# edantec/MPC_benchmark

Hardware: AMD Instinct MI355X
Metric: mpc_solves_per_sec (higher is better)
Workload: dtype f64

## Files before the change

### mpc_benchmark_amd/csrc/layout.h

```cpp
#pragma once
#include <stdint.h>

struct Layout {
  int N, B, space, nx, n, m, c, nz;
  int nj;
  int model_mask_off;
  int oH, oG, oAB, oF, oE6, oT6k, oD12, oCV, oCD, oLO, oHI, oDT, oACT, oCT, oMISC, oXD, oWR, oXN, knot_stride;
  int oP, op, oK, ok, oKnu, oknu, oMx, omx, oT6, oPhi, ophi, gain_stride;
  int oMu, oZnu, oGam, oKu, oKnup, oLm, mpad;
  int lSg, lsg, lZx, lzc, lcP, lcp, lth, ldP, leg_stride;
  int tP, tLm, tSg, tZx, tZt, tF, tE, tp, tsg, tzc, tu, txin, ttho, tree_stride;
  int wPh, wPt, wLp, wG, wHh, wgh, wCt, wW, wY, wSc, wV, wAcl, wvec, work_stride;
  int max_stage_ints, max_stage_doubles;
  int n_alpha;
  int sc_cap;
};

enum { MISC_COST = 0, MISC_PEN = 1, MISC_PRIM = 2, MISC_NC = 3, MISC_M = 4, MISC_DUAL = 5, MISC_CRIT = 6, MISC_DMERIT = 7, MISC_COUNT = 8 };

struct InstState {
  double mu, inner_tol, prim_tol;
  double phi0, dphi0, alpha, cost, prim, dual, crit;
  int32_t num_iters, al_iters, converged, done, skip_step, ls_step, ls_more, stalled;
  int32_t corrector, pad_;
// ... 6 lines not shown
static inline void make_layout(Layout& L) {
  const int n = L.n, m = L.m, c = L.c, nz = L.nz = n + m;
  int o = 0;
  auto take = [&](int cnt) { int r = o; o += align2(cnt); return r; };
  L.oH = take(nz * nz); L.oG = take(nz); L.oAB = take(n * nz); L.oF = take(n); L.oE6 = take(36); L.oT6k = take(36);
  L.oD12 = take(74);
  L.oCV = take(c); L.oCD = take(c * nz); L.oLO = take(c); L.oHI = take(c); L.oDT = take(c); L.oACT = take(c); L.oCT = take(c);
  L.oMISC = take(MISC_COUNT); L.oXD = take(n); L.oWR = take(12); L.oXN = take(L.nx);
  L.knot_stride = o;
  o = 0;
  L.oP = take(n * n); L.op = take(n); L.oK = take(m * n); L.ok = take(m); L.oKnu = take(c * n); L.oknu = take(c);
  L.oMx = take(n * n); L.omx = take(n); L.oT6 = take(36);
  L.oPhi = take(n * n); L.ophi = take(n);
  L.mpad = (m + 15) & ~15;
  L.oMu = take(L.mpad * L.mpad); L.oZnu = take(c * L.mpad); L.oGam = take(n * n); L.oKu = take(m * n); L.oKnup = take(c * n); L.oLm = take(n * n);
  L.gain_stride = o;
  o = 0;
  L.lSg = take(n * n); L.lsg = take(n); L.lZx = take(n * n); L.lzc = take(n); L.lcP = take(n * n); L.lcp = take(n); L.lth = take(n); L.ldP = take(n * n);
  L.leg_stride = o;
  o = 0;
  L.tP = take(n * n); L.tLm = take(n * n); L.tSg = take(n * n); L.tZx = take(n * n); L.tZt = take(n * n); L.tF = take(n * n); L.tE = take(n * n);
  L.tp = take(n); L.tsg = take(n); L.tzc = take(n); L.tu = take(n); L.txin = take(n); L.ttho = take(n);
  L.tree_stride = o;
  o = 0;
  const int nr = n + 1;
  L.wPh = take(n * n); L.wPt = take(n * n); L.wLp = take(n * n); L.wG = take(n * nz); L.wHh = take(nz * nz); L.wgh = take(nz);
  L.wCt = take(c * nz); L.wW = take(m * nr); L.wY = take(m * c); L.wSc = take(c * c); L.wV = take(c * nr); L.wAcl = take(n * nr);
  L.wvec = take(8 * (nz + c));
  L.work_stride = o;
  L.sc_cap = c < 48 ? c : 48;
// ... 2 lines not shown
```

### mpc_benchmark_amd/csrc/legs.h

```cpp
#pragma once
#include "mfma_blocks.h"
#include "solver_kernels.h"

#define LEG_BARRIER() asm volatile("s_waitcnt lgkmcnt(0)\n\ts_barrier" ::: "memory")

#define LEG_LAUNDER() do { asm volatile("" : "+v"(tid), "+v"(lane)); wv = __builtin_amdgcn_readfirstlane(tid >> 6); } while (0)

#define LK_THREADS 512
#define LK_U 20
#define LK_PT 13
#define LK_TILES 5

struct LkLds {
  int np, mp, nzp, lda, ldp, ldm, nb, nbm;
  int AB, PR, TM, ZN, vec, total_bytes;
  unsigned mg_nzp, mg_np, mg_mp;
};
static inline constexpr LkLds make_lk_lds(int n, int m) {
  LkLds s{};
  s.np = (n + 15) & ~15; s.mp = (m + 15) & ~15; s.nzp = s.np + s.mp; s.lda = s.nzp + 1; s.ldp = s.np + 1; s.ldm = s.mp + 1;
  s.nb = s.np / 16; s.nbm = s.mp / 16;
  s.mg_nzp = magic_div(s.nzp); s.mg_np = magic_div(s.np); s.mg_mp = magic_div(s.mp);
  int o = 0;
  auto take = [&](int cnt) { int r = o; o += (cnt + 1) & ~1; return r; };
  const int pr = s.np * s.ldp > s.mp * s.np + s.mp * s.ldm ? s.np * s.ldp : s.mp * s.np + s.mp * s.ldm;
  s.AB = take(s.np * s.lda); s.PR = take(pr); s.TM = take(6 * s.nzp + 6 * s.np + 40); s.ZN = take(16 * s.ldm); s.vec = take(s.mp + 3 * s.np + 80 + 8);
  s.total_bytes = o * 8;
  return s;
}

template <int MP, int FN = 0, int FM = 0>
DEV void leg_knot_body(const SolverArgs& a, const LkLds& Srt, const int b, const int kbeg, const int kend, const int prof_b, const int prof_k) {
  constexpr bool FX = FN > 0;
  constexpr LkLds SC_ = FX ? make_lk_lds(FN, FM) : LkLds{};
  LkLds S_ = Srt;
  if constexpr (FX) S_ = SC_;
  const LkLds& S = S_;
  constexpr int NAB = (80 * (80 + MP) + LK_THREADS - 1) / LK_THREADS, NK = (MP * 80 + LK_THREADS - 1) / LK_THREADS;
  constexpr int NMU = (MP * MP + LK_THREADS - 1) / LK_THREADS, NZN = (16 * MP + LK_THREADS - 1) / LK_THREADS;
  const Layout& L = a.L;
  int tid = threadIdx.x, lane = tid & 63;
  constexpr int nthr = LK_THREADS, nw = LK_THREADS / 64;
  int wv = __builtin_amdgcn_readfirstlane(tid >> 6);
  const InstState& st = a.inst[b];
  if (st.done || st.skip_step) return;
  const int n = FX ? FN : L.n, nz = FX ? FN + FM : L.nz, np = S.np, mp = S.mp, nzp = S.nzp, lda = S.lda, ldp = S.ldp, ldm = S.ldm, nb = S.nb, nbm = S.nbm;
  const double mud = st.mu * a.opt.dyn_al_scale;
  extern __shared__ __attribute__((aligned(16))) double sm[];
  double *AB = sm + S.AB, *PR = sm + S.PR, *ZN = sm + S.ZN, *vec = sm + S.vec;
  double *KM = PR, *PT = PR, *U1 = PR, *MU = PR + mp * np;
  double *TMP = sm + S.TM, *PT6 = TMP + 6 * nzp, *c6 = PT6 + 6 * np;
  double *kf = vec, *y0 = vec + mp, *z0 = y0 + np, *t6 = z0 + np, *g6 = t6 + 36, *mxs = g6 + 36;
  int* cnt = (int*)(mxs + np);
  long long tk0_ = clock64();
#define LK_PROF(slot) do { if (a.prof && k == prof_k && b == prof_b && tid == 0) { const long long t1_ = clock64(); a.prof[prof_b * 64 + 32 + (slot)] += (double)(t1_ - tk0_); tk0_ = t1_; } } while (0)

  double pab[NAB], pkm[NK], ptv[LK_PT], pmu[NMU], pzn[NZN], psm = 0.0, pact = 0.0;
  auto request_ab = [&](int k) {
    const double* kn = knot_ptr(a, b, k);
    const double* g = gain_ptr(a, b, k);
    const int m = (int)kn[L.oMISC + MISC_M], c = (int)kn[L.oMISC + MISC_NC];
#pragma unroll
    for (int u = 0; u < NAB; ++u) {
      const int idx = tid + u * nthr, i = qdiv(idx, S.mg_nzp), zp = (idx - qdiv(idx, S.mg_nzp) * nzp);
      const int z = (zp < n) ? zp : ((zp >= np && zp - np < m) ? n + zp - np : -1);
      pab[u] = (idx < np * nzp && i < n && z >= 0) ? kn[L.oAB + (size_t)i * nz + z] : 0.0;
    }
#pragma unroll
    for (int u = 0; u < NK; ++u) {
      const int idx = tid + u * nthr, l = qdiv(idx, S.mg_np), j = (idx - qdiv(idx, S.mg_np) * np);
      pkm[u] = (idx < mp * np && l < m && j < n) ? g[L.oK + l * n + j] : 0.0;
    }
    psm = (tid < mp) ? ((tid < m) ? g[L.ok + tid] : 0.0) : ((tid >= 64 && tid < 100) ? g[L.oT6 + tid - 64] : ((tid >= 128 && tid < 128 + n) ? g[L.omx + tid - 128] : 0.0));
    pact = (tid < c) ? kn[L.oACT + tid] : 0.0;
  };
  auto request_pt = [&](int k) {
    const double* g = gain_ptr(a, b, k);
#pragma unroll
    for (int u = 0; u < LK_PT; ++u) {
      const int idx = tid + u * nthr, i = qdiv(idx, S.mg_np), j = (idx - qdiv(idx, S.mg_np) * np);
      ptv[u] = (idx < np * np && i < n && j < n) ? g[L.oMx + i * n + j] : 0.0;
// ... 7 lines not shown
    for (int u = 0; u < NZN; ++u) { const int idx = tid + u * nthr; pzn[u] = (idx < 16 * mp) ? g[L.oZnu + idx] : 0.0; }
  };

  request_ab(kbeg);
  request_pt(kbeg);
  if (leg_of_knot(a, kbeg) + 1 < a.nlegs) request_mu(kbeg);
  for (int k = kbeg; k < kend; ++k) {
    const double* kn = knot_ptr(a, b, k);
    double* g = gain_ptr(a, b, k);
    const int m = (int)kn[L.oMISC + MISC_M];
    const bool par = leg_of_knot(a, k) + 1 < a.nlegs;
    const bool more = k + 1 < kend, par_next = more && leg_of_knot(a, k + 1) + 1 < a.nlegs;
    LEG_BARRIER();
    LEG_LAUNDER();
    if (a.prof) tk0_ = clock64();
#pragma unroll
    for (int u = 0; u < NAB; ++u) { const int idx = tid + u * nthr; if (idx < np * nzp) AB[(qdiv(idx, S.mg_nzp)) * lda + (idx - qdiv(idx, S.mg_nzp) * nzp)] = pab[u]; }
#pragma unroll
    for (int u = 0; u < NK; ++u) { const int idx = tid + u * nthr; if (idx < mp * np) KM[idx] = pkm[u]; }
    if (tid < mp) kf[tid] = psm;
    else if (tid >= 64 && tid < 100) t6[tid - 64] = psm;
    else if (tid >= 128 && tid < 128 + np) mxs[tid - 128] = psm;
    int ca = 0;
    if (par) {
      const unsigned long long act = __ballot(pact != 0.0);
      if (lane == 0) cnt[wv] = __popcll(act);
    }
    LEG_BARRIER();
    if (par) for (int w = 0; w < nw; ++w) ca += cnt[w];
    LEG_LAUNDER();
    if (more) request_ab(k + 1);
    LEG_LAUNDER();
    LK_PROF(0);
    for (int t = wv; t < nb * nb; t += nw) {
      const int ri = t / nb, cj = t % nb;
      double* At = AB + (ri * 16) * lda + cj * 16;
      d4_t acc = tile_load(At, lda, lane);
      mma_tile<false>(acc, AB + (ri * 16) * lda + np, lda, 1, KM + cj * 16, np, 1, mp, lane);
      tile_store(At, lda, acc, lane);
    }
    for (int i = wv; i < np; i += nw) {
      double s = (lane < m) ? AB[i * lda + np + lane] * kf[lane] : 0.0;
      s = wave_sum(s);
      if (lane == 0) y0[i] = s + mxs[i];
    }
    if (tid < 36) { const int i = tid / 6, j = tid % 6; double s = 0; for (int l = 0; l < 6; ++l) s += t6[i * 6 + l] * t6[j * 6 + l]; g6[tid] = s; }
    LEG_BARRIER();
    LEG_LAUNDER();
#pragma unroll
    for (int u = 0; u < LK_PT; ++u) { const int idx = tid + u * nthr; if (idx < np * np) PT[(qdiv(idx, S.mg_np)) * ldp + (idx - qdiv(idx, S.mg_np) * np)] = ptv[u]; }
    LEG_BARRIER();
    LEG_LAUNDER();
    if (more) request_pt(k + 1);
    LEG_LAUNDER();
    LK_PROF(1);
    const int nct = par ? nb + nbm : nb;
    d4_t res[LK_TILES];
#pragma unroll
    for (int sidx = 0; sidx < LK_TILES; ++sidx) {
      const int t = wv + sidx * nw;
      res[sidx] = d4_t{0, 0, 0, 0};
      if (t < nb * nct) mma_tile<false>(res[sidx], PT + ((t / nct) * 16) * ldp, ldp, 1, AB + (t % nct) * 16, lda, 1, np, lane);
    }
    for (int i = wv; i < n; i += nw) {
      double s = 0;
      for (int j = lane; j < n; j += 64) s += PT[i * ldp + j] * y0[j];
      s = wave_sum(s);
      if (lane == 0) z0[i] = y0[i] - mud * s;
    }
    LEG_BARRIER();
#pragma unroll
    for (int sidx = 0; sidx < LK_TILES; ++sidx) {
      const int t = wv + sidx * nw;
      if (t < nb * nct) {
        double* At = AB + ((t / nct) * 16) * lda + (t % nct) * 16;
        const int row = lane >> 4, col = lane & 15;
#pragma unroll
        for (int q = 0; q < 4; ++q) At[(row + 4 * q) * lda + col] -= mud * res[sidx][q];
      }
    }
    LEG_BARRIER();
    LK_PROF(2);
    for (int idx = tid; idx < 6 * nzp; idx += nthr) TMP[idx] = AB[(qdiv(idx, S.mg_nzp)) * lda + (idx - qdiv(idx, S.mg_nzp) * nzp)];
    if (par) for (int idx = tid; idx < np * 6; idx += nthr) {
      const int i = idx / 6, j = idx % 6;
      double s = 0;
      for (int l = 0; l < 6; ++l) s += PT[i * ldp + l] * t6[j * 6 + l];
      PT6[idx] = s;
    }
    LEG_BARRIER();
    for (int idx = tid; idx < 6 * nzp; idx += nthr) {
      const int i = qdiv(idx, S.mg_nzp), z = (idx - qdiv(idx, S.mg_nzp) * nzp);
      double s = 0;
      for (int l = 0; l < 6; ++l) s += t6[i * 6 + l] * TMP[l * nzp + z];
      AB[i * lda + z] = s;
    }
// ... 84 lines not shown
#pragma unroll
        for (int q = 0; q < 4; ++q) {
          const int row = ri * 16 + (lane >> 4) + 4 * q;
          if (row < n && col < n) {
            const double tt = (row < 6 && col < 6) ? g6[row * 6 + col] : (row == col ? 1.0 : 0.0);
            const double tp = (row < 6 && col < 6) ? c6[row * 6 + col] : (col < 6 ? PT6[row * 6 + col] : (row < 6 ? PT6[col * 6 + row] : ptt[q]));
            g[L.oGam + row * n + col] = -acc[q] - mud * (tt - mud * tp);
          }
        }
      }
      LK_PROF(6);
    } else if (par_next) request_mu(k + 1);
  }
}

template <int MP, int FN = 0, int FM = 0>
__global__ void __launch_bounds__(LK_THREADS) k_leg_knot(SolverArgs a, LkLds Srt, int chunk, int kmax) {
  const int kbeg = blockIdx.x * chunk, kend = (kbeg + chunk < kmax) ? kbeg + chunk : kmax;
  if (kbeg < kend) leg_knot_body<MP, FN, FM>(a, Srt, blockIdx.y, kbeg, kend, 1, 1);
}

struct LcLds { int np, ldp, nb; int LM, BA, BB, vec, total_bytes; unsigned mg_np, mg_ldp; };
static inline constexpr int lc_ld(int np) { int ld = np; while ((ld & 31) != 16) ++ld; return ld; }
static inline constexpr LcLds make_lc_lds(int n) {
  LcLds s{};
  s.np = (n + 15) & ~15; s.ldp = lc_ld(s.np); s.nb = s.np / 16;
  s.mg_np = magic_div(s.np); s.mg_ldp = magic_div(s.ldp);
  int o = 0;
  auto take = [&](int cnt) { int r = o; o += (cnt + 1) & ~1; return r; };
  s.LM = take(s.np * s.ldp); s.BA = take(s.np * s.ldp); s.BB = take(s.np * s.ldp); s.vec = take(3 * s.np + 16);
  s.total_bytes = o * 8;
  return s;
}
#define LC_TILES 4
// ... 117 lines not shown
        const int row = tri[sidx] * 16 + (lane >> 4) + 4 * q;
        if (row < n && col < n) {
          if (tri[sidx] != tcj[sidx]) { lr[L.lSg + row * n + col] = sacc[sidx][q]; lr[L.lSg + col * n + row] = sacc[sidx][q]; }
          else if (col <= row) { lr[L.lSg + row * n + col] = sacc[sidx][q]; lr[L.lSg + col * n + row] = sacc[sidx][q]; }
        }
      }
    }
  for (int i = tid; i < n; i += nthr) lr[L.lsg + i] = sg[i];
}

template <int FN = 0>
__global__ void __launch_bounds__(LK_THREADS) k_leg_condense(SolverArgs a, LcLds Srt) {
  leg_condense_body<FN>(a, Srt, blockIdx.x, blockIdx.y);
}

template <int MP, int FN = 0, int FM = 0>
__global__ void __launch_bounds__(LK_THREADS) k_leg_condense_tail(SolverArgs a, LcLds Sc, LkLds Sk, int tail) {
  const int j = blockIdx.x, b = blockIdx.y;
  if (j + 1 < a.nlegs) leg_condense_body<FN>(a, Sc, j, b);
  else {
    const int kend = a.L.N, kbeg = kend - tail;
    if (kbeg >= 0 && kbeg < kend) leg_knot_body<MP, FN, FM>(a, Sk, b, kbeg, kend, -1, -1);
  }
}

struct LxLds { int np, mp, ldp, nb, nbm; int PC, MA, RB, vec, iw, total_bytes; unsigned mg_np, mg_ldp; };
static inline constexpr LxLds make_lx_lds(int n, int m) {
  LxLds s{};
  s.np = (n + 15) & ~15; s.mp = (m + 15) & ~15; s.ldp = s.np + 1; s.nb = s.np / 16; s.nbm = s.mp / 16;
  s.mg_np = magic_div(s.np); s.mg_ldp = magic_div(s.ldp);
  int o = 0;
  auto take = [&](int cnt) { int r = o; o += (cnt + 1) & ~1; return r; };
  s.PC = take(s.np * s.ldp); s.MA = take(s.np * s.ldp); s.RB = take(s.np * s.ldp);
  s.vec = take(8 * s.np + 16 + 128);
  s.iw = o;
  s.total_bytes = o * 8 + (2 * s.np + 8) * 4;
  return s;
// ... 450 lines not shown
```

### mpc_benchmark_amd/csrc/mpc_hip.hip

```cpp
#include <hip/hip_runtime.h>
#include <mutex>
#include <map>
#include <cmath>
#include <cstdio>
#include <cstdlib>
#include <cstring>
#include <limits>
#include <stdexcept>
#include <string>
#include <utility>
#include <vector>

#include "eval_multibody_host.h"
#include "eval_reuse_kernels.h"
#include "eval_vector.h"
#include "riccati_mfma.h"
#include "closed_loop.h"
#include "legs.h"
#include "legs_tree.h"
#include "pipeline_glue.h"
#include "pipeline_ikid_glue.h"
#include "pipeline_contacts.h"
#include "pipeline_fd_glue.h"
#include "sim_record.h"
// ... 147 lines not shown
  int stage_next = 0;
  RicLds ric{};
  int ric_fixed = 0;
  ClLds cl{};
  bool use_mfma_riccati = false;
  LkLds lk{};
  LcLds lc{};
  LxLds lx{};
  bool legs_ok = false;
  bool env_chain = false, env_plain = false, env_reject_failed = false;
  int env_tree_sweeps = 0, env_trace = -1;
  int env_tail_knots = -1, cu_count = 0;
  int tail_last = 0, tail_sweeps_last = 0;
  long long tail_fused = 0, tail_separate = 0;
  long long leg_passes_multi = 0, leg_passes_single = 0;
  int leg_tail_knots(int J) const {
    if (J < 2 || env_tail_knots == 0) return 0;
    const int last = L.N - (int)((long long)(J - 1) * L.N / J);
    if (env_tail_knots > 0) return env_tail_knots < last ? env_tail_knots : last;
    if ((long long)J * L.B > cu_count || (long long)L.N * L.B <= cu_count) return 0;
    const int t = 21 * (L.N / J) / 25;
    return t < last ? t : last;
  }
  int env_apply_chunk = -1;
  bool env_duals_plain = false;
  int apply_chunk_last = 0;
  long long apply_chunked = 0, apply_single = 0;
  long long duals_staged = 0, duals_plain = 0;
  int leg_apply_chunk(int J) const {
    int C;
// ... 57 lines not shown
    a.L = L; a.opt = opt; a.head = head;
    a.stage_desc = d_stage_desc; a.stage_params = d_stage_params; a.model_i = d_model_i; a.model_d = d_model_d;
    a.xs = d_xs; a.us = d_us; a.vs = d_vs; a.lams = d_lams; a.vs_e = d_vs_e; a.lams_e = d_lams_e; a.x0 = d_x0;
    a.dxs = d_dxs; a.dus = d_dus; a.dvs = d_dvs; a.dlams = d_dlams; a.abdz = nullptr;
    a.khead = khead; a.spec = d_spec; a.isolate = isolate ? 1 : 0; a.inst_params = d_inst_params;
    const bool mpc_tick = tick_reuse && opt.max_iters <= 4 && L.space == MPC_SPACE_MULTIBODY;
    a.spec_on = (mpc_tick && !(spec_skip_pass && pass_in_run >= opt.max_iters - 1)) ? 1 : 0;
    a.reuse_on = (mpc_tick && reuse_this_pass && !(spec_skip_pass && pass_in_run == 0)) ? 1 : 0;
    a.reuse_k0 = perfect_feedback ? 1 : 0;
    a.reuse_same = (a.reuse_on && reuse_same_now) ? 1 : 0;
    a.spec_knot = a.spec_on ? d_spec_knot : nullptr; a.spec_next = (a.reuse_on && spec_next_now) ? 1 : 0;
    for (int w = 0; w < MPC_DIRTY_WORDS; ++w) a.dirty[w] = a.reuse_on ? dirty_now[w] : 0ull;
    a.only_knot = only_knot;
    a.corrector_on = corrector_armed() ? 1 : 0;
    a.reject_failed = env_reject_failed ? 1 : 0;
    a.tree_pivoted = getenv("MPC_HIP_TREE_PIVOTED") ? 1 : 0;
    a.nlegs = eff_legs(); a.leg_cap = leg_cap; a.legbuf = d_legbuf; a.treebuf = d_treebuf; a.leg_guess = leg_guess_now;
    a.knots = d_knots; a.gains = d_gains; a.work = d_work; a.trial_phi = d_trial_phi; a.inst = d_inst; a.all_done = d_all_done; a.prof = phase_timers ? d_prof : nullptr;
    return a;
  }
  size_t riccati_lds() const {
    return ((size_t)L.n * L.n + (size_t)L.m * L.m + (size_t)L.sc_cap * L.sc_cap) * sizeof(double) + ((size_t)L.c + 4) * sizeof(int);
  }
};

static void copy_sync(mpc_solver* s, void* dst, const void* src, size_t bytes, hipMemcpyKind kind) {
  HIP_OK(hipMemcpyAsync(dst, src, bytes, kind, s->stream));
  HIP_OK(hipStreamSynchronize(s->stream));
}

// ... 18 lines not shown
  s->leg_cap = need;
  s->leg_guess_valid = false;
  HIP_OK(hipStreamSynchronize(s->stream));
}

static void create_impl(mpc_solver* s, const mpc_dims& d) {
  s->dims = d;
  { const char* e;
    e = getenv("MPC_LEGS_CHAIN"); s->env_chain = e && atoi(e) > 0;
    e = getenv("MPC_LEGS_PLAIN"); s->env_plain = e && atoi(e) > 0;
    e = getenv("MPC_HIP_REJECT_FAILED"); s->env_reject_failed = e && atoi(e) > 0;
    e = getenv("MPC_TREE_SWEEPS"); s->env_tree_sweeps = e ? atoi(e) : 0;
    e = getenv("MPC_HIP_TRACE"); s->env_trace = e ? atoi(e) : -1;
    e = getenv("MPC_LEG_TAIL_KNOTS"); s->env_tail_knots = e ? (atoi(e) > 0 ? atoi(e) : 0) : -1;
    e = getenv("MPC_LEG_APPLY_CHUNK"); s->env_apply_chunk = (e && atoi(e) > 0) ? atoi(e) : -1;
    e = getenv("MPC_DUALS_PLAIN"); s->env_duals_plain = e && atoi(e) > 0; }
  HIP_OK(hipSetDevice(d.device));
  HIP_OK(hipDeviceGetAttribute(&s->cu_count, hipDeviceAttributeMultiprocessorCount, d.device));
  { const char* e = getenv("MPC_LEG_TAIL_CUS"); if (e && atoi(e) > 0) s->cu_count = atoi(e); }
  {
    static int created = 0;
    const char* pe = getenv("MPC_HIP_STREAM_PRIO");
    if (pe && atoi(pe) > 0) {
      int lo = 0, hi = 0;
      HIP_OK(hipDeviceGetStreamPriorityRange(&lo, &hi));
      const int levels = lo - hi + 1;
      const int prio = hi + (created++ % levels);
      HIP_OK(hipStreamCreateWithPriority(&s->stream, hipStreamNonBlocking, prio));
      if (atoi(pe) > 1) fprintf(stderr, "[mpc] stream priority %d (range %d..%d)\n", prio, hi, lo);
    } else {
// ... 76 lines not shown
  s->lk = make_lk_lds(L.n, L.m); s->lc = make_lc_lds(L.n); s->lx = make_lx_lds(L.n, L.m);
  s->legs_ok = s->use_mfma_riccati && s->ric.np <= 80 && s->ric.mp <= 48 && L.c <= 256 && s->ric.gfull >= 1 && s->lk.total_bytes <= 160 * 1024 &&
               s->lc.total_bytes <= 160 * 1024 && s->lx.total_bytes <= 160 * 1024 && !getenv("MPC_HIP_NO_LEGS");
  if (s->legs_ok) {
    lds_attr_max((const void*)k_riccati_mfma<RIC_THREADS, 80, true, true>, s->ric.total_bytes);
    s->ric_fixed = 0;
    if (!getenv("MPC_HIP_GENERIC_DIMS") && s->ric.sq) {
#define X(ID, FN, FM, GF, ST, NPV, MPV) if (!s->ric_fixed && L.n == FN && L.m == FM && L.nz == FN + FM && ric_same_layout(s->ric, ric_fixed_layout(FN, FM, true, GF, ST))) s->ric_fixed = ID;
      MPC_FIXED_MODELS(X)
#undef X
    }
    const int leg_tail_lds = s->lc.total_bytes > s->lk.total_bytes ? s->lc.total_bytes : s->lk.total_bytes;
#define X(ID, FN, FM, GF, ST, NPV, MPV) if (s->ric_fixed == ID) { \
      lds_attr_max((const void*)k_riccati_mfma<RIC_THREADS, 80, true, true, FN, FM, GF, ST>, s->ric.total_bytes); \
      lds_attr_max((const void*)k_leg_knot<MPV, FN, FM>, s->lk.total_bytes); \
      lds_attr_max((const void*)k_leg_condense<FN>, s->lc.total_bytes); \
      lds_attr_max((const void*)k_leg_condense_tail<MPV, FN, FM>, leg_tail_lds); \
      lds_attr_max((const void*)k_leg_compose<NPV, FN, FM>, s->lx.total_bytes); \
      lds_attr_max((const void*)k_leg_tree_down<NPV, FN, FM>, s->lx.total_bytes); }
    MPC_FIXED_MODELS(X)
#undef X
    lds_attr_max((const void*)k_riccati_mfma<RIC_THREADS, 80, false, true>, s->ric.total_bytes);
    lds_attr_max((const void*)k_riccati_mfma<RIC_SMALL_THREADS, 16, false, true>, s->ric.total_bytes);
    lds_attr_max((const void*)k_leg_knot<16>, s->lk.total_bytes);
    lds_attr_max((const void*)k_leg_knot<32>, s->lk.total_bytes);
    lds_attr_max((const void*)k_leg_knot<48>, s->lk.total_bytes);
    lds_attr_max((const void*)k_leg_condense<0>, s->lc.total_bytes);
    lds_attr_max((const void*)k_leg_condense_tail<16>, leg_tail_lds);
    lds_attr_max((const void*)k_leg_condense_tail<32>, leg_tail_lds);
    lds_attr_max((const void*)k_leg_condense_tail<48>, leg_tail_lds);
// ... 234 lines not shown
      MPC_FIXED_MODELS(X)
#undef X
      else if (s->ric.sq) hipLaunchKernelGGL(HIP_KERNEL_NAME(k_riccati_mfma<RIC_THREADS, 80, true, true>), dim3(L.B * J), dim3(RIC_THREADS), s->ric.total_bytes, s->stream, a, s->ric);
      else hipLaunchKernelGGL(HIP_KERNEL_NAME(k_riccati_mfma<RIC_THREADS, 80, false, true>), dim3(L.B * J), dim3(RIC_THREADS), s->ric.total_bytes, s->stream, a, s->ric);
    }
    else if (s->use_mfma_riccati && s->ric.np == 16 && s->ric.mp == 16 && L.c <= RIC_SMALL_THREADS)
      hipLaunchKernelGGL(HIP_KERNEL_NAME(k_riccati_mfma<RIC_SMALL_THREADS, 16>), dim3(L.B), dim3(RIC_SMALL_THREADS), s->ric.total_bytes, s->stream, a, s->ric);
    else if (s->use_mfma_riccati && s->ric.sq && s->ric.np <= 80) hipLaunchKernelGGL(HIP_KERNEL_NAME(k_riccati_mfma<RIC_THREADS, 80, true>), dim3(L.B), dim3(RIC_THREADS), s->ric.total_bytes, s->stream, a, s->ric);
    else if (s->use_mfma_riccati && s->ric.sq) hipLaunchKernelGGL(HIP_KERNEL_NAME(k_riccati_mfma<RIC_THREADS, 96, true>), dim3(L.B), dim3(RIC_THREADS), s->ric.total_bytes, s->stream, a, s->ric);
    else if (s->use_mfma_riccati && s->ric.np <= 80) hipLaunchKernelGGL(HIP_KERNEL_NAME(k_riccati_mfma<RIC_THREADS, 80>), dim3(L.B), dim3(RIC_THREADS), s->ric.total_bytes, s->stream, a, s->ric);
    else if (s->use_mfma_riccati) hipLaunchKernelGGL(HIP_KERNEL_NAME(k_riccati_mfma<RIC_THREADS, 96>), dim3(L.B), dim3(RIC_THREADS), s->ric.total_bytes, s->stream, a, s->ric);
    else hipLaunchKernelGGL(k_riccati_backward, dim3(L.B), dim3(256), s->riccati_lds(), s->stream, a);
  });
  if (J > 1) {
    s->timed(12, "k_closed_loop", [&] {
      static const int chunk_env = getenv("MPC_LEG_KNOT_CHUNK") ? atoi(getenv("MPC_LEG_KNOT_CHUNK")) : 0;
      const int chunk = chunk_env > 0 ? chunk_env : 1;
      const int kmax = L.N - tail;
      const dim3 grid((kmax + chunk - 1) / chunk, L.B);
      if (false) {}
#define X(ID, FN, FM, GF, ST, NPV, MPV) else if (s->ric_fixed == ID) hipLaunchKernelGGL((k_leg_knot<MPV, FN, FM>), grid, dim3(LK_THREADS), s->lk.total_bytes, s->stream, a, s->lk, chunk, kmax);
      MPC_FIXED_MODELS(X)
#undef X
      else if (s->lk.mp <= 16) hipLaunchKernelGGL(k_leg_knot<16>, grid, dim3(LK_THREADS), s->lk.total_bytes, s->stream, a, s->lk, chunk, kmax);
      else if (s->lk.mp <= 32) hipLaunchKernelGGL(k_leg_knot<32>, grid, dim3(LK_THREADS), s->lk.total_bytes, s->stream, a, s->lk, chunk, kmax);
      else hipLaunchKernelGGL(k_leg_knot<48>, grid, dim3(LK_THREADS), s->lk.total_bytes, s->stream, a, s->lk, chunk, kmax);
    });
    if (tail > 0) s->timed(13, "k_leg_condense", [&] {
      const int lds = s->lc.total_bytes > s->lk.total_bytes ? s->lc.total_bytes : s->lk.total_bytes;
      const dim3 grid(J, L.B);
      s->tail_fused++;
      if (false) {}
#define X(ID, FN, FM, GF, ST, NPV, MPV) else if (s->ric_fixed == ID) hipLaunchKernelGGL((k_leg_condense_tail<MPV, FN, FM>), grid, dim3(LK_THREADS), lds, s->stream, a, s->lc, s->lk, tail);
      MPC_FIXED_MODELS(X)
#undef X
      else if (s->lk.mp <= 16) hipLaunchKernelGGL(k_leg_condense_tail<16>, grid, dim3(LK_THREADS), lds, s->stream, a, s->lc, s->lk, tail);
      else if (s->lk.mp <= 32) hipLaunchKernelGGL(k_leg_condense_tail<32>, grid, dim3(LK_THREADS), lds, s->stream, a, s->lc, s->lk, tail);
      else hipLaunchKernelGGL(k_leg_condense_tail<48>, grid, dim3(LK_THREADS), lds, s->stream, a, s->lc, s->lk, tail);
    });
    else s->timed(13, "k_leg_condense", [&] {
      s->tail_separate++;
      if (false) {}
#define X(ID, FN, FM, GF, ST, NPV, MPV) else if (s->ric_fixed == ID) hipLaunchKernelGGL(k_leg_condense<FN>, dim3(J - 1, L.B), dim3(LK_THREADS), s->lc.total_bytes, s->stream, a, s->lc);
      MPC_FIXED_MODELS(X)
#undef X
      else hipLaunchKernelGGL(k_leg_condense<0>, dim3(J - 1, L.B), dim3(LK_THREADS), s->lc.total_bytes, s->stream, a, s->lc);
    });
    if (tree) s->timed(14, "k_leg_consensus", [&] {
// ... 943 lines not shown
      if (!s->d_legbuf || k >= s->leg_cap - 1) throw std::runtime_error("debug_get: no such leg record");
      const double* lr = s->d_legbuf + ((size_t)b * (s->leg_cap - 1) + k) * L.leg_stride;
      if (nm == "Sg") dev_vec(lr + L.lSg, n * n); else if (nm == "sg") dev_vec(lr + L.lsg, n); else if (nm == "Zx") dev_vec(lr + L.lZx, n * n);
      else if (nm == "zc") dev_vec(lr + L.lzc, n); else if (nm == "calP") dev_vec(lr + L.ldP, n * n);
      else if (nm == "calp") dev_vec(lr + L.lcp, n);
      else dev_vec(lr + L.lth, n);
    }
    else if (nm == "ls_knot") {
      std::vector<double> tp((size_t)L.n_alpha * (L.N + 1));
      copy_sync(s, tp.data(), s->d_trial_phi + (size_t)b * L.n_alpha * (L.N + 1), tp.size() * sizeof(double), hipMemcpyDeviceToHost);
      for (int i = 0; i < L.n_alpha; ++i) v.push_back(tp[(size_t)i * (L.N + 1) + k]);
      v.push_back(kn[L.oMISC + MISC_COST]); v.push_back(kn[L.oMISC + MISC_PEN]);
    }
    else if (nm == "leg_tail") v = {(double)s->tail_last, (double)s->tail_fused, (double)s->tail_separate, (double)s->tail_sweeps_last, (double)s->eff_legs(), (double)s->cu_count,
                                   (double)s->leg_passes_multi, (double)s->leg_passes_single};
    else if (nm == "backsubst") v = {(double)s->apply_chunk_last, (double)s->apply_chunked, (double)s->apply_single, (double)s->duals_staged, (double)s->duals_plain,
                                    (double)leg_apply_chunks(L.N, s->eff_legs(), s->apply_chunk_last > 0 ? s->apply_chunk_last : 1)};
    else if (nm == "fixed_dims") v = {(double)s->ric_fixed};
    else if (nm == "ric_prof") { dev_vec(s->d_prof + (size_t)b * 64, 64); HIP_OK(hipMemsetAsync(s->d_prof + (size_t)b * 64, 0, 64 * sizeof(double), s->stream)); HIP_OK(hipStreamSynchronize(s->stream)); }
    else if (nm == "dx") dev_vec(s->d_dxs + ((size_t)b * (L.N + 1) + k) * n, n);
    else if (nm == "du") { if (k >= L.N) throw std::runtime_error("no du at the terminal knot"); dev_vec(s->d_dus + ((size_t)b * L.N + k) * L.m, L.m); }
    else if (nm == "dvs") dev_vec(s->d_dvs + ((size_t)b * (L.N + 1) + k) * L.c, L.c);
    else if (nm == "dlams") dev_vec(s->d_dlams + ((size_t)b * (L.N + 1) + k) * n, n);
    else throw std::runtime_error("debug_get: unknown quantity " + nm);
    if ((int)v.size() > cap) throw std::runtime_error("debug_get: output buffer too small");
    if (!v.empty()) std::memcpy(out, v.data(), v.size() * sizeof(double));
    return (int)v.size();
  } catch (const std::exception& e) {
    s->err = e.what();
    return -1;
// ... 10 lines not shown
```

### mpc_benchmark_amd/csrc/riccati_mfma.h

```cpp
#pragma once
#include "solver_kernels.h"
#include "mfma_blocks.h"

#ifndef RIC_SMALL_THREADS
#define RIC_SMALL_THREADS 256
#endif
#ifndef RIC_THREADS
#define RIC_THREADS 512
#endif
#if RIC_THREADS <= 256
#define RIC_WAVES_ATTR __attribute__((amdgpu_waves_per_eu(1, 1)))
#else
#define RIC_WAVES_ATTR
#endif
#define RIC_MAX_SERIES 8
#define RIC_SERIES_TOL 1e-14

#define RIC_LAUNDER() do { asm volatile("" : "+v"(tid), "+v"(lane)); wv = __builtin_amdgcn_readfirstlane(tid >> 6); } while (0)
#define RIC_SQ_DIMS() int n_l_ = n; asm volatile("" : "+s"(n_l_)); const int nv = SQ ? (n_l_ >> 1) : 0, ks = SQ ? (nv & ~3) : 0, Ke = SQ ? ((n_l_ + 3) & ~3) - ks : np; (void)nv; (void)ks; (void)Ke
#ifndef RIC_PROF_TID
#define RIC_PROF_TID 0
#endif
#ifdef RIC_SUBPROF
#define RIC_SUB(slot) RIC_PROF(slot)
// ... 543 lines not shown
        if (t < ngt) {
          const int ri = t / nzt, cj = t % nzt;
          if (sq && cj * 16 < nv) {
            const int col = cj * 16 + (lane & 15);
#pragma unroll
            for (int q = 0; q < 4; ++q) {
              const int row = ri * 16 + (lane >> 4) + 4 * q;
              double ad = 0.0;
              if (col >= 6) ad = (col < nv) ? PT[row * ldp + col] : 0.0;
              else for (int l = 0; l < 6; ++l) ad += PT[row * ldp + l] * d12l[l * 6 + col];
              gres[sidx][q] += ad;
            }
          }
          if (cj < nb) tile_store(PT + (ri * 16) * ldp + cj * 16, ldp, gres[sidx], lane);
          else tile_store(GU + (ri * 16) * mp + (cj - nb) * 16, mp, gres[sidx], lane);
        }
      }
      __syncthreads();
      RIC_SUB(27);
      const int nht = nzt * (nzt + 1) / 2, nxt = nb * (nb + 1) / 2;
      auto hh_tile_at = [&](int zi, int cj, d4_t& out, int (&zr)[4], int& zc, const double* hp) {
        const int col_p = cj * 16 + (lane & 15);
        zc = (col_p < n) ? col_p : ((col_p >= np && col_p - np < m) ? n + col_p - np : -1);
        double h[4];
#pragma unroll
        for (int q = 0; q < 4; ++q) {
          const int rp = zi * 16 + (lane >> 4) + 4 * q;
          zr[q] = (rp < n) ? rp : ((rp >= np && rp - np < m) ? n + rp - np : -1);
          h[q] = hp ? hp[q] : kn[L.oH + (zr[q] >= 0 ? zr[q] : 0) * nz + (zc >= 0 ? zc : 0)] * ((zr[q] >= 0 && zc >= 0) ? 1.0 : 0.0);
        }
// ... 472 lines not shown
```

### mpc_benchmark_amd/csrc/solver_args.h

```cpp
#pragma once
#include "device_common.h"

#define MPC_STALL_TOL 1e-13

#define MPC_DIRTY_WORDS 4

struct SolverArgs {
  Layout L;
  mpc_options opt;
  int head;
  const int32_t* stage_desc;
  const double* stage_params;
  const double* inst_params;
  const int32_t* model_i;
  const double* model_d;
  double *xs, *us, *vs, *lams, *vs_e, *lams_e, *x0;
  double *dxs, *dus, *dvs, *dlams;
  int isolate;
  int khead;
  int spec_on;
  int reuse_on;
  int reuse_k0;
  int reuse_same;
  int* spec;
// ... 2 lines not shown
  double *trial_phi;
  InstState* inst;
  int* all_done;
  double* prof;
  int nlegs;
  int leg_cap;
  int leg_guess;
  double* legbuf;
  double* treebuf;
  double* spec_knot;
  int spec_next;
  unsigned long long dirty[MPC_DIRTY_WORDS];
  int only_knot;
  int corrector_on;
  int reject_failed;
  int tree_pivoted;
};

DEV int leg_start(const SolverArgs& a, int j) { return (int)((long long)j * a.L.N / a.nlegs); }
DEV int leg_of_knot(const SolverArgs& a, int k) { int j = a.nlegs - 1; while (j > 0 && leg_start(a, j) > k) --j; return j; }
DEV double* leg_ptr(const SolverArgs& a, int b, int j) { return a.legbuf + ((size_t)b * (a.leg_cap - 1) + j) * a.L.leg_stride; }

DEV int knot_slot(const SolverArgs& a, int k) { return k < a.L.N ? (a.khead + k) % a.L.N : a.L.N; }
DEV double* knot_ptr(const SolverArgs& a, int b, int k) { return a.knots + ((size_t)b * (a.L.N + 1) + knot_slot(a, k)) * a.L.knot_stride; }
DEV bool knot_reused(const SolverArgs& a, int b, int k) {
  if (!(a.reuse_on && a.spec[b])) return false;
  if ((a.dirty[(k >> 6) & (MPC_DIRTY_WORDS - 1)] >> (k & 63)) & 1ull) return false;
  if (a.reuse_same) return true;
  if (k < a.L.N - 1) return k > 0 || a.reuse_k0;
  return a.spec_next != 0 && a.spec[b] == 1;
// ... 41 lines not shown
```

Baseline: 12320.

## Add opt-in G-matrix closed-loop knot form and auto-select leg knot chunk

Stores a G·AB product from the Riccati kernel into a new gain slot. An optional leg-knot variant then builds the closed-loop matrix from q/v halves with a small 6x6 correction, instead of the full tiled MFMA product. That variant only runs when MPC_LEG_KNOT_G is set. Separately, the knot chunk size is now picked by a heuristic that minimises knots per CU wave, replacing the fixed default of 1. This changes grid size and per-block work in the default path.

After: 12370, median of 6. No clear change (+0.4%).

```diff
diff --git a/mpc_benchmark_amd/csrc/layout.h b/mpc_benchmark_amd/csrc/layout.h
--- a/mpc_benchmark_amd/csrc/layout.h
+++ b/mpc_benchmark_amd/csrc/layout.h
@@ -8,6 +8,7 @@
   int oH, oG, oAB, oF, oE6, oT6k, oD12, oCV, oCD, oLO, oHI, oDT, oACT, oCT, oMISC, oXD, oWR, oXN, knot_stride;
   int oP, op, oK, ok, oKnu, oknu, oMx, omx, oT6, oPhi, ophi, gain_stride;
   int oMu, oZnu, oGam, oKu, oKnup, oLm, mpad;
+  int oGab;
   int lSg, lsg, lZx, lzc, lcP, lcp, lth, ldP, leg_stride;
   int tP, tLm, tSg, tZx, tZt, tF, tE, tp, tsg, tzc, tu, txin, ttho, tree_stride;
   int wPh, wPt, wLp, wG, wHh, wgh, wCt, wW, wY, wSc, wV, wAcl, wvec, work_stride;
@@ -44,6 +45,7 @@
   L.oPhi = take(n * n); L.ophi = take(n);
   L.mpad = (m + 15) & ~15;
   L.oMu = take(L.mpad * L.mpad); L.oZnu = take(c * L.mpad); L.oGam = take(n * n); L.oKu = take(m * n); L.oKnup = take(c * n); L.oLm = take(n * n);
+  L.oGab = take(n * nz);
   L.gain_stride = o;
   o = 0;
   L.lSg = take(n * n); L.lsg = take(n); L.lZx = take(n * n); L.lzc = take(n); L.lcP = take(n * n); L.lcp = take(n); L.lth = take(n); L.ldP = take(n * n);
diff --git a/mpc_benchmark_amd/csrc/legs.h b/mpc_benchmark_amd/csrc/legs.h
--- a/mpc_benchmark_amd/csrc/legs.h
+++ b/mpc_benchmark_amd/csrc/legs.h
@@ -11,32 +11,18 @@
 #define LK_PT 13
 #define LK_TILES 5
 
-struct LkLds {
-  int np, mp, nzp, lda, ldp, ldm, nb, nbm;
-  int AB, PR, TM, ZN, vec, total_bytes;
-  unsigned mg_nzp, mg_np, mg_mp;
-};
-static inline constexpr LkLds make_lk_lds(int n, int m) {
-  LkLds s{};
-  s.np = (n + 15) & ~15; s.mp = (m + 15) & ~15; s.nzp = s.np + s.mp; s.lda = s.nzp + 1; s.ldp = s.np + 1; s.ldm = s.mp + 1;
-  s.nb = s.np / 16; s.nbm = s.mp / 16;
-  s.mg_nzp = magic_div(s.nzp); s.mg_np = magic_div(s.np); s.mg_mp = magic_div(s.mp);
-  int o = 0;
-  auto take = [&](int cnt) { int r = o; o += (cnt + 1) & ~1; return r; };
-  const int pr = s.np * s.ldp > s.mp * s.np + s.mp * s.ldm ? s.np * s.ldp : s.mp * s.np + s.mp * s.ldm;
-  s.AB = take(s.np * s.lda); s.PR = take(pr); s.TM = take(6 * s.nzp + 6 * s.np + 40); s.ZN = take(16 * s.ldm); s.vec = take(s.mp + 3 * s.np + 80 + 8);
-  s.total_bytes = o * 8;
-  return s;
-}
-
-template <int MP, int FN = 0, int FM = 0>
+#include "legs_layout.h"
+
+template <int MP, int FN = 0, int FM = 0, bool GH = false>
 DEV void leg_knot_body(const SolverArgs& a, const LkLds& Srt, const int b, const int kbeg, const int kend, const int prof_b, const int prof_k) {
   constexpr bool FX = FN > 0;
   constexpr LkLds SC_ = FX ? make_lk_lds(FN, FM) : LkLds{};
   LkLds S_ = Srt;
   if constexpr (FX) S_ = SC_;
   const LkLds& S = S_;
-  constexpr int NAB = (80 * (80 + MP) + LK_THREADS - 1) / LK_THREADS, NK = (MP * 80 + LK_THREADS - 1) / LK_THREADS;
+  static_assert(!GH || (FN > 0 && FN % 2 == 0 && FN >= 12), "the G form needs compile-time dimensions with q and v halves");
+  constexpr int NVH = FN / 2;
+  constexpr int NAB = GH ? 1 : (80 * (80 + MP) + LK_THREADS - 1) / LK_THREADS, NGH = GH ? (NVH * SC_.nzp + LK_THREADS - 1) / LK_THREADS : 1, NK = (MP * 80 + LK_THREADS - 1) / LK_THREADS;
   constexpr int NMU = (MP * MP + LK_THREADS - 1) / LK_THREADS, NZN = (16 * MP + LK_THREADS - 1) / LK_THREADS;
   const Layout& L = a.L;
   int tid = threadIdx.x, lane = tid & 63;
@@ -47,24 +33,41 @@
   const int n = FX ? FN : L.n, nz = FX ? FN + FM : L.nz, np = S.np, mp = S.mp, nzp = S.nzp, lda = S.lda, ldp = S.ldp, ldm = S.ldm, nb = S.nb, nbm = S.nbm;
   const double mud = st.mu * a.opt.dyn_al_scale;
   extern __shared__ __attribute__((aligned(16))) double sm[];
-  double *AB = sm + S.AB, *PR = sm + S.PR, *ZN = sm + S.ZN, *vec = sm + S.vec;
+  double *AB = sm + S.AB, *PR = sm + S.PR, *ZN = sm + S.ZN;
   double *KM = PR, *PT = PR, *U1 = PR, *MU = PR + mp * np;
-  double *TMP = sm + S.TM, *PT6 = TMP + 6 * nzp, *c6 = PT6 + 6 * np;
-  double *kf = vec, *y0 = vec + mp, *z0 = y0 + np, *t6 = z0 + np, *g6 = t6 + 36, *mxs = g6 + 36;
-  int* cnt = (int*)(mxs + np);
+  const LkSub SU = make_lk_sub(S);
+  double *TMP = sm + SU.tmp, *PT6 = sm + SU.pt6, *c6 = sm + SU.c6;
+  double *kf = sm + SU.kf, *y0 = sm + SU.y0, *z0 = sm + SU.z0, *t6 = sm + SU.t6, *g6 = sm + SU.g6, *mxs = sm + SU.mxs;
+  int* cnt = (int*)(sm + SU.cnt);
   long long tk0_ = clock64();
 #define LK_PROF(slot) do { if (a.prof && k == prof_k && b == prof_b && tid == 0) { const long long t1_ = clock64(); a.prof[prof_b * 64 + 32 + (slot)] += (double)(t1_ - tk0_); tk0_ = t1_; } } while (0)
 
   double pab[NAB], pkm[NK], ptv[LK_PT], pmu[NMU], pzn[NZN], psm = 0.0, pact = 0.0;
+  double pabq[NGH], pabv[NGH], pgq[NGH], pgv[NGH], pddb = 0.0, pdt = 0.0;
   auto request_ab = [&](int k) {
     const double* kn = knot_ptr(a, b, k);
     const double* g = gain_ptr(a, b, k);
     const int m = (int)kn[L.oMISC + MISC_M], c = (int)kn[L.oMISC + MISC_NC];
+    if constexpr (GH) {
+#pragma unroll
+      for (int u = 0; u < NGH; ++u) {
+        const int idx = tid + u * nthr, jq = qdiv(idx, S.mg_nzp), zp = (idx - qdiv(idx, S.mg_nzp) * nzp);
+        const int z = (zp < n) ? zp : ((zp >= np && zp - np < m) ? n + zp - np : -1);
+        const bool ok = idx < NVH * nzp && z >= 0;
+        const int off = ok ? jq * nz + z : 0;
+        const double msk = ok ? 1.0 : 0.0;
+        pabq[u] = kn[L.oAB + off] * msk; pabv[u] = kn[L.oAB + NVH * nz + off] * msk;
+        pgq[u] = g[L.oGab + off] * msk; pgv[u] = g[L.oGab + NVH * nz + off] * msk;
+      }
+      pddb = kn[L.oD12 + 36 + (tid < 36 ? tid : 0)];
+      pdt = kn[L.oD12 + 72];
+    } else {
 #pragma unroll
     for (int u = 0; u < NAB; ++u) {
       const int idx = tid + u * nthr, i = qdiv(idx, S.mg_nzp), zp = (idx - qdiv(idx, S.mg_nzp) * nzp);
       const int z = (zp < n) ? zp : ((zp >= np && zp - np < m) ? n + zp - np : -1);
       pab[u] = (idx < np * nzp && i < n && z >= 0) ? kn[L.oAB + (size_t)i * nz + z] : 0.0;
+    }
     }
 #pragma unroll
     for (int u = 0; u < NK; ++u) {
@@ -102,8 +105,25 @@
     LEG_BARRIER();
     LEG_LAUNDER();
     if (a.prof) tk0_ = clock64();
+    if constexpr (GH) {
+#pragma unroll
+      for (int u = 0; u < NGH; ++u) {
+        const int idx = tid + u * nthr;
+        if (idx < NVH * nzp) {
+          const int jq = qdiv(idx, S.mg_nzp), zp = idx - jq * nzp;
+          const double mg = mud * pgq[u];
+          double mv = pabv[u] - mud * pgv[u];
+          if (jq >= 6) mv += pdt * mg; else TMP[jq * nzp + zp] = mg;
+          AB[jq * lda + zp] = pabq[u] - mg;
+          AB[(NVH + jq) * lda + zp] = mv;
+        }
+      }
+      for (int idx = tid; idx < (np - n) * nzp; idx += nthr) AB[(n + qdiv(idx, S.mg_nzp)) * lda + (idx - qdiv(idx, S.mg_nzp) * nzp)] = 0.0;
+      if (tid < 36) PT6[tid] = pddb;
+    } else {
 #pragma unroll
     for (int u = 0; u < NAB; ++u) { const int idx = tid + u * nthr; if (idx < np * nzp) AB[(qdiv(idx, S.mg_nzp)) * lda + (idx - qdiv(idx, S.mg_nzp) * nzp)] = pab[u]; }
+    }
 #pragma unroll
     for (int u = 0; u < NK; ++u) { const int idx = tid + u * nthr; if (idx < mp * np) KM[idx] = pkm[u]; }
     if (tid < mp) kf[tid] = psm;
@@ -120,6 +140,17 @@
     if (more) request_ab(k + 1);
     LEG_LAUNDER();
     LK_PROF(0);
+    if constexpr (GH) {
+      for (int idx = tid; idx < 6 * nzp; idx += nthr) {
+        const int jq = qdiv(idx, S.mg_nzp), zp = idx - jq * nzp;
+        double s = 0;
+#pragma unroll
+        for (int l = 0; l < 6; ++l) s += PT6[l * 6 + jq] * TMP[l * nzp + zp];
+        AB[(NVH + jq) * lda + zp] += s;
+      }
+      LEG_BARRIER();
+      LEG_LAUNDER();
+    }
     for (int t = wv; t < nb * nb; t += nw) {
       const int ri = t / nb, cj = t % nb;
       double* At = AB + (ri * 16) * lda + cj * 16;
@@ -130,7 +161,7 @@
     for (int i = wv; i < np; i += nw) {
       double s = (lane < m) ? AB[i * lda + np + lane] * kf[lane] : 0.0;
       s = wave_sum(s);
-      if (lane == 0) y0[i] = s + mxs[i];
+      if (lane == 0) y0[i] = GH ? s : s + mxs[i];
     }
     if (tid < 36) { const int i = tid / 6, j = tid % 6; double s = 0; for (int l = 0; l < 6; ++l) s += t6[i * 6 + l] * t6[j * 6 + l]; g6[tid] = s; }
     LEG_BARRIER();
@@ -142,6 +173,14 @@
     if (more) request_pt(k + 1);
     LEG_LAUNDER();
     LK_PROF(1);
+    if constexpr (GH) {
+      for (int i = wv; i < n; i += nw) {
+        double s = 0;
+        for (int j = lane; j < n; j += 64) s += PT[i * ldp + j] * mxs[j];
+        s = wave_sum(s);
+        if (lane == 0) z0[i] = y0[i] + mxs[i] - mud * s;
+      }
+    } else {
     const int nct = par ? nb + nbm : nb;
     d4_t res[LK_TILES];
 #pragma unroll
@@ -168,6 +207,7 @@
       }
     }
     LEG_BARRIER();
+    }
     LK_PROF(2);
     for (int idx = tid; idx < 6 * nzp; idx += nthr) TMP[idx] = AB[(qdiv(idx, S.mg_nzp)) * lda + (idx - qdiv(idx, S.mg_nzp) * nzp)];
     if (par) for (int idx = tid; idx < np * 6; idx += nthr) {
@@ -282,10 +322,10 @@
   }
 }
 
-template <int MP, int FN = 0, int FM = 0>
+template <int MP, int FN = 0, int FM = 0, bool GH = false>
 __global__ void __launch_bounds__(LK_THREADS) k_leg_knot(SolverArgs a, LkLds Srt, int chunk, int kmax) {
   const int kbeg = blockIdx.x * chunk, kend = (kbeg + chunk < kmax) ? kbeg + chunk : kmax;
-  if (kbeg < kend) leg_knot_body<MP, FN, FM>(a, Srt, blockIdx.y, kbeg, kend, 1, 1);
+  if (kbeg < kend) leg_knot_body<MP, FN, FM, GH>(a, Srt, blockIdx.y, kbeg, kend, 1, 1);
 }
 
 struct LcLds { int np, ldp, nb; int LM, BA, BB, vec, total_bytes; unsigned mg_np, mg_ldp; };
@@ -433,13 +473,13 @@
   leg_condense_body<FN>(a, Srt, blockIdx.x, blockIdx.y);
 }
 
-template <int MP, int FN = 0, int FM = 0>
+template <int MP, int FN = 0, int FM = 0, bool GH = false>
 __global__ void __launch_bounds__(LK_THREADS) k_leg_condense_tail(SolverArgs a, LcLds Sc, LkLds Sk, int tail) {
   const int j = blockIdx.x, b = blockIdx.y;
   if (j + 1 < a.nlegs) leg_condense_body<FN>(a, Sc, j, b);
   else {
     const int kend = a.L.N, kbeg = kend - tail;
-    if (kbeg >= 0 && kbeg < kend) leg_knot_body<MP, FN, FM>(a, Sk, b, kbeg, kend, -1, -1);
+    if (kbeg >= 0 && kbeg < kend) leg_knot_body<MP, FN, FM, GH>(a, Sk, b, kbeg, kend, -1, -1);
   }
 }
 
diff --git a/mpc_benchmark_amd/csrc/legs_layout.h b/mpc_benchmark_amd/csrc/legs_layout.h
--- /dev/null
+++ b/mpc_benchmark_amd/csrc/legs_layout.h
@@ -0,0 +1,31 @@
+#pragma once
+#ifndef RIC_MAGIC_DIV_DEFINED
+#define RIC_MAGIC_DIV_DEFINED
+static inline constexpr unsigned ric_magic_div(int d) { return (unsigned)((0x100000000ull + (unsigned long long)d - 1) / (unsigned long long)d); }
+#endif
+
+struct LkLds {
+  int np, mp, nzp, lda, ldp, ldm, nb, nbm;
+  int AB, PR, TM, ZN, vec, total_bytes;
+  unsigned mg_nzp, mg_np, mg_mp;
+};
+static inline constexpr LkLds make_lk_lds(int n, int m) {
+  LkLds s{};
+  s.np = (n + 15) & ~15; s.mp = (m + 15) & ~15; s.nzp = s.np + s.mp; s.lda = s.nzp + 1; s.ldp = s.np + 1; s.ldm = s.mp + 1;
+  s.nb = s.np / 16; s.nbm = s.mp / 16;
+  s.mg_nzp = ric_magic_div(s.nzp); s.mg_np = ric_magic_div(s.np); s.mg_mp = ric_magic_div(s.mp);
+  int o = 0;
+  auto take = [&](int cnt) { int r = o; o += (cnt + 1) & ~1; return r; };
+  const int pr = s.np * s.ldp > s.mp * s.np + s.mp * s.ldm ? s.np * s.ldp : s.mp * s.np + s.mp * s.ldm;
+  s.AB = take(s.np * s.lda); s.PR = take(pr); s.TM = take(6 * s.nzp + 6 * s.np + 40); s.ZN = take(16 * s.ldm); s.vec = take(s.mp + 3 * s.np + 80 + 8);
+  s.total_bytes = o * 8;
+  return s;
+}
+
+struct LkSub { int tmp, pt6, c6, tm_end, kf, y0, z0, t6, g6, mxs, cnt, vec_end; };
+static inline constexpr LkSub make_lk_sub(const LkLds& s) {
+  LkSub u{};
+  u.tmp = s.TM; u.pt6 = u.tmp + 6 * s.nzp; u.c6 = u.pt6 + 6 * s.np; u.tm_end = u.c6 + 36;
+  u.kf = s.vec; u.y0 = u.kf + s.mp; u.z0 = u.y0 + s.np; u.t6 = u.z0 + s.np; u.g6 = u.t6 + 36; u.mxs = u.g6 + 36; u.cnt = u.mxs + s.np; u.vec_end = u.cnt + 4;
+  return u;
+}
diff --git a/mpc_benchmark_amd/csrc/mpc_hip.hip b/mpc_benchmark_amd/csrc/mpc_hip.hip
--- a/mpc_benchmark_amd/csrc/mpc_hip.hip
+++ b/mpc_benchmark_amd/csrc/mpc_hip.hip
@@ -185,6 +185,28 @@
   int tail_last = 0, tail_sweeps_last = 0;
   long long tail_fused = 0, tail_separate = 0;
   long long leg_passes_multi = 0, leg_passes_single = 0;
+  bool env_knot_g = false;
+  int env_knot_chunk = 0;
+  int knot_chunk_last = 0;
+  int leg_knot_chunk(int kmax) const {
+    if (env_knot_chunk > 0) return env_knot_chunk;
+    const int cus = cu_count > 0 ? cu_count : 1;
+    int best = 1;
+    long long best_knots = -1;
+    for (int C = 1; C <= 10; ++C) {
+      const long long wgs = (long long)((kmax + C - 1) / C) * L.B, knots = ((wgs + cus - 1) / cus) * C;
+      if (best_knots < 0 || knots <= best_knots) { if (best_knots < 0 || knots < best_knots || C > best) best = C; best_knots = knots; }
+    }
+    return best;
+  }
+  long long knot_g = 0, knot_plain = 0;
+  bool leg_knot_g() const {
+    if (!env_knot_g || !legs_ok) return false;
+#define X(ID, FN, FM, GF, ST, NPV, MPV) if (ric_fixed == ID) return MPV <= 32;
+    MPC_FIXED_MODELS(X)
+#undef X
+    return false;
+  }
   int leg_tail_knots(int J) const {
     if (J < 2 || env_tail_knots == 0) return 0;
     const int last = L.N - (int)((long long)(J - 1) * L.N / J);
@@ -272,6 +294,7 @@
     a.only_knot = only_knot;
     a.corrector_on = corrector_armed() ? 1 : 0;
     a.reject_failed = env_reject_failed ? 1 : 0;
+    a.leg_gab = (leg_knot_g() && eff_legs() > 1) ? 1 : 0;
     a.tree_pivoted = getenv("MPC_HIP_TREE_PIVOTED") ? 1 : 0;
     a.nlegs = eff_legs(); a.leg_cap = leg_cap; a.legbuf = d_legbuf; a.treebuf = d_treebuf; a.leg_guess = leg_guess_now;
     a.knots = d_knots; a.gains = d_gains; a.work = d_work; a.trial_phi = d_trial_phi; a.inst = d_inst; a.all_done = d_all_done; a.prof = phase_timers ? d_prof : nullptr;
@@ -320,6 +343,8 @@
     e = getenv("MPC_HIP_TRACE"); s->env_trace = e ? atoi(e) : -1;
     e = getenv("MPC_LEG_TAIL_KNOTS"); s->env_tail_knots = e ? (atoi(e) > 0 ? atoi(e) : 0) : -1;
     e = getenv("MPC_LEG_APPLY_CHUNK"); s->env_apply_chunk = (e && atoi(e) > 0) ? atoi(e) : -1;
+    e = getenv("MPC_LEG_KNOT_G"); s->env_knot_g = e && atoi(e) > 0;
+    e = getenv("MPC_LEG_KNOT_CHUNK"); s->env_knot_chunk = e ? atoi(e) : 0;
     e = getenv("MPC_DUALS_PLAIN"); s->env_duals_plain = e && atoi(e) > 0; }
   HIP_OK(hipSetDevice(d.device));
   HIP_OK(hipDeviceGetAttribute(&s->cu_count, hipDeviceAttributeMultiprocessorCount, d.device));
@@ -426,6 +451,8 @@
 #define X(ID, FN, FM, GF, ST, NPV, MPV) if (s->ric_fixed == ID) { \
       lds_attr_max((const void*)k_riccati_mfma<RIC_THREADS, 80, true, true, FN, FM, GF, ST>, s->ric.total_bytes); \
       lds_attr_max((const void*)k_leg_knot<MPV, FN, FM>, s->lk.total_bytes); \
+      lds_attr_max((const void*)k_leg_knot<MPV, FN, FM, (MPV <= 32)>, s->lk.total_bytes); \
+      lds_attr_max((const void*)k_leg_condense_tail<MPV, FN, FM, (MPV <= 32)>, leg_tail_lds); \
       lds_attr_max((const void*)k_leg_condense<FN>, s->lc.total_bytes); \
       lds_attr_max((const void*)k_leg_condense_tail<MPV, FN, FM>, leg_tail_lds); \
       lds_attr_max((const void*)k_leg_compose<NPV, FN, FM>, s->lx.total_bytes); \
@@ -690,12 +717,14 @@
   });
   if (J > 1) {
     s->timed(12, "k_closed_loop", [&] {
-      static const int chunk_env = getenv("MPC_LEG_KNOT_CHUNK") ? atoi(getenv("MPC_LEG_KNOT_CHUNK")) : 0;
-      const int chunk = chunk_env > 0 ? chunk_env : 1;
       const int kmax = L.N - tail;
+      const int chunk = s->leg_knot_chunk(kmax);
+      s->knot_chunk_last = chunk;
       const dim3 grid((kmax + chunk - 1) / chunk, L.B);
+      if (a.leg_gab) s->knot_g++; else s->knot_plain++;
       if (false) {}
-#define X(ID, FN, FM, GF, ST, NPV, MPV) else if (s->ric_fixed == ID) hipLaunchKernelGGL((k_leg_knot<MPV, FN, FM>), grid, dim3(LK_THREADS), s->lk.total_bytes, s->stream, a, s->lk, chunk, kmax);
+#define X(ID, FN, FM, GF, ST, NPV, MPV) else if (s->ric_fixed == ID && a.leg_gab) hipLaunchKernelGGL((k_leg_knot<MPV, FN, FM, (MPV <= 32)>), grid, dim3(LK_THREADS), s->lk.total_bytes, s->stream, a, s->lk, chunk, kmax); \
+      else if (s->ric_fixed == ID) hipLaunchKernelGGL((k_leg_knot<MPV, FN, FM>), grid, dim3(LK_THREADS), s->lk.total_bytes, s->stream, a, s->lk, chunk, kmax);
       MPC_FIXED_MODELS(X)
 #undef X
       else if (s->lk.mp <= 16) hipLaunchKernelGGL(k_leg_knot<16>, grid, dim3(LK_THREADS), s->lk.total_bytes, s->stream, a, s->lk, chunk, kmax);
@@ -707,7 +736,8 @@
       const dim3 grid(J, L.B);
       s->tail_fused++;
       if (false) {}
-#define X(ID, FN, FM, GF, ST, NPV, MPV) else if (s->ric_fixed == ID) hipLaunchKernelGGL((k_leg_condense_tail<MPV, FN, FM>), grid, dim3(LK_THREADS), lds, s->stream, a, s->lc, s->lk, tail);
+#define X(ID, FN, FM, GF, ST, NPV, MPV) else if (s->ric_fixed == ID && a.leg_gab) hipLaunchKernelGGL((k_leg_condense_tail<MPV, FN, FM, (MPV <= 32)>), grid, dim3(LK_THREADS), lds, s->stream, a, s->lc, s->lk, tail); \
+      else if (s->ric_fixed == ID) hipLaunchKernelGGL((k_leg_condense_tail<MPV, FN, FM>), grid, dim3(LK_THREADS), lds, s->stream, a, s->lc, s->lk, tail);
       MPC_FIXED_MODELS(X)
 #undef X
       else if (s->lk.mp <= 16) hipLaunchKernelGGL(k_leg_condense_tail<16>, grid, dim3(LK_THREADS), lds, s->stream, a, s->lc, s->lk, tail);
@@ -1681,6 +1711,8 @@
     }
     else if (nm == "leg_tail") v = {(double)s->tail_last, (double)s->tail_fused, (double)s->tail_separate, (double)s->tail_sweeps_last, (double)s->eff_legs(), (double)s->cu_count,
                                    (double)s->leg_passes_multi, (double)s->leg_passes_single};
+    else if (nm == "leg_knot_form") v = {(double)s->knot_g, (double)s->knot_plain, s->leg_knot_g() ? 1.0 : 0.0, (double)s->knot_chunk_last};
+    else if (nm == "Gab") mat(g.data() + L.oGab, k < L.N ? n : 0, nz, nz);
     else if (nm == "backsubst") v = {(double)s->apply_chunk_last, (double)s->apply_chunked, (double)s->apply_single, (double)s->duals_staged, (double)s->duals_plain,
                                     (double)leg_apply_chunks(L.N, s->eff_legs(), s->apply_chunk_last > 0 ? s->apply_chunk_last : 1)};
     else if (nm == "fixed_dims") v = {(double)s->ric_fixed};
diff --git a/mpc_benchmark_amd/csrc/riccati_mfma.h b/mpc_benchmark_amd/csrc/riccati_mfma.h
--- a/mpc_benchmark_amd/csrc/riccati_mfma.h
+++ b/mpc_benchmark_amd/csrc/riccati_mfma.h
@@ -581,6 +581,16 @@
           }
           if (cj < nb) tile_store(PT + (ri * 16) * ldp + cj * 16, ldp, gres[sidx], lane);
           else tile_store(GU + (ri * 16) * mp + (cj - nb) * 16, mp, gres[sidx], lane);
+          if constexpr (LEGS && FX && SQ) {
+            if (a.leg_gab) {
+              const int zc = (cj < nb) ? cj * 16 + (lane & 15) : n + (cj - nb) * 16 + (lane & 15);
+              if (zc < ((cj < nb) ? n : nz)) {
+                double* go = g + L.oGab + zc;
+#pragma unroll
+                for (int q = 0; q < 4; ++q) { const int row = ri * 16 + (lane >> 4) + 4 * q; if (row < n) go[row * nz] = gres[sidx][q]; }
+              }
+            }
+          }
         }
       }
       __syncthreads();
diff --git a/mpc_benchmark_amd/csrc/solver_args.h b/mpc_benchmark_amd/csrc/solver_args.h
--- a/mpc_benchmark_amd/csrc/solver_args.h
+++ b/mpc_benchmark_amd/csrc/solver_args.h
@@ -40,6 +40,7 @@
   int only_knot;
   int corrector_on;
   int reject_failed;
+  int leg_gab;
   int tree_pivoted;
 };
 
```
